# aviadlevis/bhnerf

Hardware: AMD Instinct MI355X
Metric: train ray-samples/sec, 128x128x64-sample image-plane recovery (higher is better)
Workload: dtype bf16

## Files before the change

bhnerf_amd/csrc/fused_bwd.hip:

```cpp
#include <climits>
#include <utility>
#include <type_traits>
#include "fused_common.h"
#include "bwd_common.h"

static constexpr int JOB1_W = 13;
static constexpr int JOBL_W = 7;
static constexpr int GA0C_DIST = 4;
static constexpr int TAPED_DIST = 7;
static constexpr int T8_NBUF = 4;

template <int W, class Pol>
struct BwdGeom {
    static constexpr int MT = W / 32;
    static constexpr int TILE_BYTES = 2 * Pol::FRAG_BYTES;
    static constexpr int TAPE_TILE = Pol::TAPE8 ? 1024 : TILE_BYTES;
    static constexpr int NTMAX = MT + 2;
    static constexpr int SLAB_FLOATS = (MT + 1) * NTMAX * 1024;
    static constexpr int WR = (MT >= 4) ? 4 : MT;
    static constexpr int WC = Pol::NWAVES / WR >= 1 ? Pol::NWAVES / WR : 1;
    static constexpr int WRR = (Pol::NWAVES < WR) ? Pol::NWAVES : WR;
    static constexpr int WCC = Pol::NWAVES / WRR;
    static constexpr int MPW = (MT + WRR - 1) / WRR;
    static constexpr int NPW_ALL = (NTMAX + WCC - 1) / WCC;
    static constexpr int SWEEP = (Pol::NWAVES <= 4) ? NTMAX : 5;
    static constexpr int NPASS = (NPW_ALL + SWEEP - 1) / SWEEP;
    static constexpr int NPW = (NPW_ALL + NPASS - 1) / NPASS;
    static constexpr int GROUP_BYTES = Pol::TAPE8 ? MT * TAPE_TILE + (MT + 1) * TILE_BYTES : (2 * MT + 1) * TILE_BYTES;
    static constexpr int GROUP_BYTES_LAST2 = GROUP_BYTES + 1024;
    static constexpr int RING_DIST_TAPED = (Pol::ELEM_BYTES == 2) ? TAPED_DIST : 3;
    static constexpr int NBUF = (Pol::ELEM_BYTES == 2) ? ((160 * 1024) / GROUP_BYTES >= 4 ? 4 : 3) : 2;
    static constexpr int NPIECE = GROUP_BYTES / 1024;
    static constexpr int PPW = (NPIECE + Pol::NWAVES - 1) / Pol::NWAVES;
};

enum { EMIT_NO_STORE = 1,
       EMIT_OFF = 2 };
template <class Pol>
struct TapeEmit {
    static constexpr int LDS_BYTES = 2 * Pol::FRAG_BYTES;
    const char *table;
    DEVI void init(char *lds) {
        table = lds;
        if (Pol::ELEM_BYTES != 2 && threadIdx.x < 64) {
            const int lane = threadIdx.x, n = lane & 31, h = lane >> 5;
            typename Pol::frag id[2];
#pragma unroll
            for (int s = 0; s < 2; ++s) {
#pragma unroll
                for (int j = 0; j < 8; ++j) Pol::set(id[s], j, phi16(h, j) + 16 * s == n ? 1.f : 0.f);
                if constexpr (Pol::ELEM_BYTES == 2) {
                    *reinterpret_cast<typename Pol::frag *>(lds + s * Pol::FRAG_BYTES + lane * 16) = id[s];
                } else {
#pragma unroll
                    for (int hf = 0; hf < 2; ++hf) {
                        f32x4 v;
#pragma unroll
                        for (int e = 0; e < 4; ++e) v[e] = Pol::get(id[s], 4 * hf + e);
                        *reinterpret_cast<f32x4 *>(lds + s * Pol::FRAG_BYTES + hf * 1024 + lane * 16) = v;
                    }
                }
            }
        }
    }
    DEVI void load_id(typename Pol::frag (&id)[2]) const {
        const int lane = threadIdx.x & 63;
        id[0] = Pol::lds_frag(table, 0, lane);
        id[1] = Pol::lds_frag(table, 1, lane);
    }
    static DEVI f32x16 transpose(const typename Pol::frag &f0, const typename Pol::frag &f1, const typename Pol::frag (&id)[2]) {
        f32x16 t = {};
        t = Pol::mma(f0, id[0], t);
        t = Pol::mma(f1, id[1], t);
        return t;
    }
    static DEVI void store(char *dst, const f32x16 &t) {
        const int lane = threadIdx.x & 63;
        typename Pol::frag o[2];
#pragma unroll
        for (int s = 0; s < 2; ++s)
#pragma unroll
            for (int j = 0; j < 8; ++j) Pol::set(o[s], j, t[8 * s + j]);
        if constexpr (Pol::ELEM_BYTES == 2) {
#pragma unroll
            for (int s = 0; s < 2; ++s) __builtin_nontemporal_store(o[s], reinterpret_cast<typename Pol::frag *>(dst + s * 1024 + lane * 16));
        } else {
#pragma unroll
            for (int s = 0; s < 2; ++s)
#pragma unroll
                for (int hf = 0; hf < 2; ++hf) {
                    f32x4 v;
#pragma unroll
                    for (int e = 0; e < 4; ++e) v[e] = Pol::get(o[s], 4 * hf + e);
                    __builtin_nontemporal_store(v, reinterpret_cast<f32x4 *>(dst + s * 2048 + hf * 1024 + lane * 16));
                }
        }
    }
    static DEVI int native_off(int s) {
        const int lane = threadIdx.x & 63, pt = lane & 31, h = lane >> 5;
        return 16 * (pt & 3) + 128 * s + 64 * h + 256 * (pt >> 2);
    }
    static DEVI void store_native(char *dst, const typename Pol::frag &f0, const typename Pol::frag &f1, int flags = 0) {
        if (!(flags & EMIT_NO_STORE)) {
            __builtin_nontemporal_store(f0, reinterpret_cast<typename Pol::frag *>(dst + native_off(0)));
            __builtin_nontemporal_store(f1, reinterpret_cast<typename Pol::frag *>(dst + native_off(1)));
        } else asm volatile("" ::"v"(f0), "v"(f1));
    }
    DEVI void emit(char *dst, const typename Pol::frag &f0, const typename Pol::frag &f1) const {
        if constexpr (Pol::ELEM_BYTES == 2) {
            store_native(dst, f0, f1);
        } else {
            typename Pol::frag id[2];
            load_id(id);
            store(dst, transpose(f0, f1, id));
        }
    }
};

DEVI long long uniform64(long long v) {
    const unsigned lo = __builtin_amdgcn_readfirstlane((unsigned)v), hi = __builtin_amdgcn_readfirstlane((unsigned)((unsigned long long)v >> 32));
    return (long long)(((unsigned long long)hi << 32) | lo);
}

DEVI int tr_lane_off() {
    const int lane = threadIdx.x & 63, g = lane >> 4, li = lane & 15, q = li >> 2, pp = li & 3;
    return 256 * (g >> 1) + 16 * q + 128 * (g & 1) + 64 * (pp & 1) + 8 * (pp >> 1);
}
DEVI bf16x8 tr_frag(const char *tile, int s, int trl) {
    typedef s16x4 __attribute__((address_space(3))) * lds_v4;
    typedef short s16x8 __attribute__((ext_vector_type(8)));
    const char *a = tile + 1024 * s + trl;
    const s16x4 lo = __builtin_amdgcn_ds_read_tr16_b64_v4i16((lds_v4)(a));
    const s16x4 hi = __builtin_amdgcn_ds_read_tr16_b64_v4i16((lds_v4)(a + 512));
    const s16x8 v = __builtin_shufflevector(lo, hi, 0, 1, 2, 3, 4, 5, 6, 7);
    return __builtin_bit_cast(bf16x8, v);
}

struct Raw8 { u32x2 lo, hi; };
DEVI int tr8_lane_off() {
    const int lane = threadIdx.x & 63, g = lane >> 4, li = lane & 15, tsel = g & 1, kh = g >> 1;
    return 1024 * tsel + 128 * (kh ^ tsel) + 32 * (li >> 2) + 8 * (li & 3);
}
DEVI Raw8 tr8_read(const char *pair, int s2, int tr8) {
    typedef s16x4 __attribute__((address_space(3))) * lds_v4;
    Raw8 r;
    r.lo = __builtin_bit_cast(u32x2, __builtin_amdgcn_ds_read_tr16_b64_v4i16((lds_v4)(pair + 512 * s2 + tr8)));
    r.hi = __builtin_bit_cast(u32x2, __builtin_amdgcn_ds_read_tr16_b64_v4i16((lds_v4)(pair + 512 * s2 + 256 + tr8)));
    return r;
}
struct Pair8 { u32x2 a, b; };
DEVI Pair8 tr8_sort(const Raw8 &r) {
    Pair8 p;
    p.a = (u32x2){__builtin_amdgcn_perm(r.lo[1], r.lo[0], 0x06040200u), __builtin_amdgcn_perm(r.hi[1], r.hi[0], 0x06040200u)};
    p.b = (u32x2){__builtin_amdgcn_perm(r.lo[1], r.lo[0], 0x07050301u), __builtin_amdgcn_perm(r.hi[1], r.hi[0], 0x07050301u)};
    return p;
}
DEVI bf16x8 widen8(const u32x2 &f, float scale) {
    typedef __bf16 b2 __attribute__((ext_vector_type(2)));
    const b2 a0 = __builtin_amdgcn_cvt_scalef32_pk_bf16_fp8(f[0], scale, false), a1 = __builtin_amdgcn_cvt_scalef32_pk_bf16_fp8(f[0], scale, true);
    const b2 a2 = __builtin_amdgcn_cvt_scalef32_pk_bf16_fp8(f[1], scale, false), a3 = __builtin_amdgcn_cvt_scalef32_pk_bf16_fp8(f[1], scale, true);
    return (bf16x8){a0[0], a0[1], a1[0], a1[1], a2[0], a2[1], a3[0], a3[1]};
}
DEVI void tr8_widen(const Raw8 &r, float scale, bf16x8 &fa, bf16x8 &fb) {
    const Pair8 p = tr8_sort(r);
    fa = widen8(p.a, scale);
    fb = widen8(p.b, scale);
}
DEVI f32x16 mma8(const u32x2 &a, const u32x2 &b, f32x16 c) {
    return __builtin_amdgcn_mfma_f32_32x32x16_fp8_fp8(__builtin_bit_cast(long, a), __builtin_bit_cast(long, b), c, 0, 0, 0);
}
__host__ __device__ static inline int t8_feature(int t, int n) {
    const int i = n & 15, hh = i >> 3, s = (i >> 2) & 1, j = 2 * (i & 3) + (t & 1);
    return 32 * ((t & ~1) + (n >> 4)) + 16 * s + 8 * (j >> 2) + 4 * hh + (j & 3);
}

// ... 669 lines not shown
    const int wr = wv % WRR, wc = wv / WRR;
    const bool wave_works = wr * MPW < mtA;
    float *slab = A.f.slabs + (long long)blockIdx.x * BG::SLAB_FLOATS;
    constexpr int PA = out_job ? TB / 1024 : MT * TB / 1024, PH = has_h ? MT * TB / 1024 : 0, PE = has_enc ? TB / 1024 : 0;
    using Stream = TapeStream<Pol::NWAVES, PA, PH, PE, 0, OFF_H, OFF_E, 0>;
    constexpr int PPW = Stream::PPW;
    const Stream stream(srcA, strideA, srcH, (long long)MT * TB, srcE, TB, nullptr, 0, wv);

    for (int pass = 0; pass < NPASS; ++pass) {
        const int nbase = wc * NPWJ + pass * NPW;
        int boff[NPW];
#pragma unroll
        for (int ni = 0; ni < NPW; ++ni) {
            const int n = nbase + ni;
            boff[ni] = (n < nH) ? OFF_H + n * TB : (has_enc ? OFF_E : OFF_H);
        }
        const bool has_tiles = nbase < nB;
        const bool bias_rows = wc == 0 && pass == 0;
        float bsum[MPW];
#pragma unroll
        for (int mi = 0; mi < MPW; ++mi) bsum[mi] = 0.f;
        f32x16 acc[MPW][NPW];
#pragma unroll
        for (int mi = 0; mi < MPW; ++mi)
#pragma unroll
            for (int ni = 0; ni < NPW; ++ni) {
                if constexpr (AGPR) {
                    const f32x16 z = {};
                    acc[mi][ni] = __builtin_amdgcn_mfma_f32_32x32x2f32(0.f, 0.f, z, 0, 0, 0);
                } else {
#pragma unroll
                    for (int r = 0; r < 16; ++r) acc[mi][ni][r] = 0.f;
                }
            }
        __syncthreads();
        auto load_b = [&](const char *gp, int t) -> frag {
            if constexpr (TR) return tr_frag(gp + boff[t % NPW], t / NPW, trl);
            else return Pol::lds_frag(gp + boff[t % NPW], t / NPW, lane);
        };
        auto load_a = [&](const char *tile, int s2) -> frag {
            if constexpr (TR) return tr_frag(tile, s2, trl);
            else return Pol::lds_frag(tile, s2, lane);
        };
        auto compute_group = [&](const char *gp) {
            constexpr int NTOT = 2 * NPW, AHEAD = (Pol::ELEM_BYTES == 2) ? 2 : 1;
            if constexpr (AGPR) {
#pragma unroll
                for (int mi = 0; mi < MPW; ++mi)
#pragma unroll
                    for (int ni = 0; ni < NPW && ni < NPIN; ++ni) asm volatile("" : "+a"(acc[mi][ni]));
            }
            frag af[2][MPW];
#pragma unroll
            for (int s = 0; s < 2; ++s)
#pragma unroll
                for (int mi = 0; mi < MPW; ++mi) {
                    af[s][mi] = load_a(gp + (wr * MPW + mi) * TB, s);
                    if (bias_rows) bsum[mi] = Pol::sum8(af[s][mi], bsum[mi]);
                }
            frag bq[AHEAD + 1];
#pragma unroll
            for (int t = 0; t < AHEAD && t < NTOT; ++t) bq[t] = load_b(gp, t);
#pragma unroll
            for (int t = 0; t < NTOT; ++t) {
                if (t + AHEAD < NTOT) bq[(t + AHEAD) % (AHEAD + 1)] = load_b(gp, t + AHEAD);
                __builtin_amdgcn_sched_barrier(0);
                const int s = t / NPW, ni = t % NPW;
                const frag bnow = bq[t % (AHEAD + 1)];
#pragma unroll
                for (int mi = 0; mi < MPW; ++mi) acc[mi][ni] = Pol::mma(af[s][mi], bnow, acc[mi][ni]);
                __builtin_amdgcn_sched_barrier(0);
            }
        };
        {
            constexpr int NBUF = BG::NBUF;
            auto issue = [&](long long q, char *buf) { stream.issue(q < q1 ? q : q1 - 1, buf); };
            constexpr int INFLIGHT = NBUF - 2;
            if (q0 < q1) {
#pragma unroll
                for (int j = 0; j < NBUF - 1; ++j) issue(q0 + j, smem + j * GB);
                int it = 0;
                for (long long q = q0; q < q1; ++q) {
                    asm volatile("s_waitcnt vmcnt(%0)" ::"n"(INFLIGHT * PPW) : "memory");
                    __builtin_amdgcn_s_barrier();
                    asm volatile("" ::: "memory");
                    const int nx = (it == 0) ? NBUF - 1 : it - 1;
                    issue(q + NBUF - 1, smem + nx * GB);
                    if (wave_works && has_tiles) compute_group(smem + it * GB);
                    it = (it == NBUF - 1) ? 0 : it + 1;
                }
                asm volatile("s_waitcnt vmcnt(0)" ::: "memory");
            }
        }
#pragma unroll
        for (int mi = 0; mi < MPW; ++mi)
#pragma unroll
            for (int ni = 0; ni < NPW; ++ni) {
                const int m = wr * MPW + mi, n = nbase + ni;
                if (m >= mtA || n >= nB || n >= (wc + 1) * NPWJ) continue;
                if constexpr (AGPR) { if (ni < NPIN) asm volatile("" : "+a"(acc[mi][ni])); }
                float *tp = slab + (long long)(m * BG::NTMAX + n) * 1024;
#pragma unroll
                for (int g4 = 0; g4 < 4; ++g4) {
                    f32x4 v;
#pragma unroll
                    for (int e = 0; e < 4; ++e) v[e] = acc[mi][ni][4 * g4 + e];
                    f32x4 *dst = reinterpret_cast<f32x4 *>(tp + g4 * 256 + lane * 4);
                    if (A.accumulate) {
                        const f32x4 old = *dst;
#pragma unroll
                        for (int e = 0; e < 4; ++e) v[e] += old[e];
                    }
                    *dst = v;
                }
                __builtin_amdgcn_sched_barrier(0);
            }
        if (bias_rows) {
#pragma unroll
            for (int mi = 0; mi < MPW; ++mi) {
                const int m = wr * MPW + mi;
                float v = bsum[mi] + __shfl_xor(bsum[mi], 32, 64);
                if (m < mtA && lane < 32) {
                    const int hh = (lane >> 2) & 1, r = (lane & 3) + 4 * (lane >> 3);
                    float *dst = slab + (long long)(m * BG::NTMAX + nB) * 1024 + (r >> 2) * 256 + (32 * hh) * 4 + (r & 3);
                    if (A.accumulate) v += *dst;
                    *dst = v;
                }
            }
        }
    }
}


template <int W, class Pol, int JT, bool LAST = false, bool OUTENC = false>
DEVI void dw_body2(const BwdArgs &A, int job, char *smem) {
    using BG = BwdGeom<W, Pol>;
    using frag = typename Pol::frag;
    static_assert(Pol::ELEM_BYTES == 2 && JT != JT_OUT && JT != JT_OUTSKIP, "bf16 jobs of layers 0 .. depth-1");
    static_assert(!LAST || JT == JT_HIDDEN || JT == JT_SKIP, "LAST: hidden / skip job");
    static_assert(!OUTENC || LAST, "OUTENC: a LAST job");
    static_assert(BG::NBUF == 4, "ring of four group buffers");
    constexpr int MT = BG::MT, TB = BG::TILE_BYTES, TT = BG::TAPE_TILE;
    constexpr bool T8 = Pol::TAPE8;
    constexpr bool has_h = JT != JT_FIRST, make_h = JT == JT_HIDDEN1, enc_extra = JT == JT_SKIP;
    static_assert(!T8 || !OUTENC, "8-bit tape: even depths / no skip into the output layer");
    constexpr int OFF_H = MT * TT, OFF_E = T8 ? OFF_H + (make_h ? MT * TB : MT * TT) : 2 * MT * TB, OFF_D32 = OFF_E + TB;
    constexpr int GB = OFF_D32 + (LAST ? 1024 : 0);
    static_assert(T8 || (OFF_D32 == BG::GROUP_BYTES && GB == (LAST ? BG::GROUP_BYTES_LAST2 : BG::GROUP_BYTES)), "group image");
    static_assert(GB <= BG::GROUP_BYTES + 1024, "group image larger than the host's LDS budget");
    constexpr int NB = (T8 && !make_h) ? T8_NBUF : 4;
    static_assert((NB & (NB - 1)) == 0 && NB >= 4 && NB * GB <= 160 * 1024, "ring size");
    constexpr int nH = has_h ? MT : 0, nB = nH + ((JT == JT_FIRST || JT == JT_SKIP) ? 1 : 0);
    constexpr int nBr = has_h ? MT : 1;
    constexpr int WRR = BG::WRR, WCC = BG::WCC;
    constexpr int MPW = (MT + WRR - 1) / WRR, NPW = (nBr + WCC - 1) / WCC;
    static_assert(NPW <= 5, "one sweep");
    constexpr bool F8 = T8 && has_h && !make_h;
    static_assert(!T8 || MPW == 2, "8-bit tape: the A tiles come in pairs (width 256)");
    static_assert(!F8 || NPW % 2 == 0, "8-bit tape: the B tiles come in pairs (width 256)");
    constexpr int ME = (MPW + WCC - 1) / WCC;
    constexpr int NTOT = 2 * NPW;
    const int tid = threadIdx.x, lane = tid & 63, wv = __builtin_amdgcn_readfirstlane(tid >> 6);
    const int trl = tr_lane_off();
    const int tr8 = tr8_lane_off();
    float scaleA = 1.f;
    if constexpr (T8 && !LAST) scaleA = __builtin_bit_cast(float, __builtin_amdgcn_readfirstlane(__builtin_bit_cast(int, A.t8[job])));
    if constexpr (F8 && LAST) {
        const float v = A.t8[job];
        scaleA = __builtin_bit_cast(float, __builtin_amdgcn_readfirstlane(__builtin_bit_cast(int, (v > 0.f && v < __builtin_inff()) ? v : 1.f)));
    }
    const int nwg = A.wg_begin[job + 1] - A.wg_begin[job];
    const int kb = blockIdx.x - A.wg_begin[job];
    const long long q0 = uniform64(A.t.NQ * kb / nwg), q1 = uniform64(A.t.NQ * (kb + 1) / nwg);
    const char *srcA = LAST ? A.tape + A.t.h_off[job + 1] : A.tape + A.t.ga_off[job];
    const char *srcD = A.tape + A.t.dout_off;
    const char *srcH = has_h ? A.tape + A.t.h_off[job] : nullptr;
    const char *srcE = A.tape + (make_h ? A.t.encp_off : A.t.enc_off);
    const int wr = wv % WRR, wc = wv / WRR;
    const int nbase = wc * NPW;
    const bool works = wr * MPW < MT && nbase < nBr;
    char *w0_lds = smem + NB * GB;
    float *b0_lds = reinterpret_cast<float *>(w0_lds + 2 * MT * Pol::FRAG_BYTES);
    if constexpr (make_h) {
        const char *w0 = A.f.packed + A.f.fwd_off;
        for (int i = tid; i < 2 * MT * Pol::FRAG_BYTES / 16; i += Pol::NTHREADS)
            reinterpret_cast<u32x4 *>(w0_lds)[i] = reinterpret_cast<const u32x4 *>(w0)[i];
        for (int i = tid; i < W; i += Pol::NTHREADS) b0_lds[i] = reinterpret_cast<const float *>(A.f.packed + A.f.bias_off)[i];
    }
    struct HIn { frag e0, e1, w0, w1; float b; };
    auto make_h_read = [&](const char *gp) {
        HIn in;
        in.e0 = Pol::lds_frag(gp + OFF_E, 0, lane); in.e1 = Pol::lds_frag(gp + OFF_E, 1, lane);
        const int t = wv < MT ? wv : 0;
        in.w0 = Pol::lds_frag(w0_lds, 2 * t, lane); in.w1 = Pol::lds_frag(w0_lds, 2 * t + 1, lane);
        in.b = b0_lds[32 * t + (lane & 31)];
        return in;
    };
    auto make_h_mma = [&](const HIn &in) {
        f32x16 acc;
#pragma unroll
        for (int r = 0; r < 16; ++r) acc[r] = in.b;
        acc = Pol::mma(in.e0, in.w0, acc);
        acc = Pol::mma(in.e1, in.w1, acc);
        return acc;
    };
    auto make_h_write = [&](char *gp, const f32x16 &acc) {
        if (wv < MT) {
            frag o[2];
            unsigned unused = 0;
#pragma unroll
            for (int r = 0; r < 16; r += 2) Pol::relu_pair(o[r >> 3], (r & 7) >> 1, r >> 1, acc[r], acc[r + 1], unused);
#pragma unroll
            for (int s2 = 0; s2 < 2; ++s2) *reinterpret_cast<frag *>(gp + OFF_H + wv * TB + s2 * Pol::FRAG_BYTES + lane * 16) = o[s2];
        }
    };
    float wout_r[MPW];
    if constexpr (LAST) {
#pragma unroll
        for (int mi = 0; mi < MPW; ++mi) {
            const int f = T8 ? t8_feature(wr * MPW + mi, lane & 31) : 32 * (wr * MPW + mi) + (lane & 31);
            wout_r[mi] = f < W ? reinterpret_cast<const float *>(A.f.packed + A.f.wout_off)[f] : 0.f;
        }
    }
    float *slab = A.f.slabs + (long long)blockIdx.x * BG::SLAB_FLOATS;

    int boff[NPW];
#pragma unroll
    for (int ni = 0; ni < NPW; ++ni) {
        const int n = nbase + ni;
        boff[ni] = has_h ? OFF_H + (n < nH ? n : 0) * (F8 ? TT : TB) : OFF_E;
    }
    const bool bias_rows = wc == 0;
    const bool out_bias_wave = LAST && wr == 0 && wc == 0;
    f32x16 acc[MPW][NPW], acc_e[ME];
    float bsum[MPW], orow[ME], bout = 0.f, oenc = 0.f;
#pragma unroll
    for (int mi = 0; mi < MPW; ++mi) {
        bsum[mi] = 0.f;
#pragma unroll
        for (int ni = 0; ni < NPW; ++ni)
#pragma unroll
            for (int r = 0; r < 16; ++r) acc[mi][ni][r] = 0.f;
    }
#pragma unroll
    for (int e = 0; e < ME; ++e) {
        orow[e] = 0.f;
#pragma unroll
        for (int r = 0; r < 16; ++r) acc_e[e][r] = 0.f;
    }

    struct AState { frag af[2][MPW]; f32x4 da[2], db[2]; frag ef[2]; u32x2 a8[2][MPW]; };
    auto load_b = [&](const char *gp, int t) -> frag {
        if constexpr (make_h) return Pol::lds_frag(gp + boff[t % NPW], t / NPW, lane);
        else return tr_frag(gp + boff[t % NPW], t / NPW, trl);
    };
    constexpr int NPH = NPW / 2 > 0 ? NPW / 2 : 1;
    auto load_braw = [&](const char *gp, int u) -> Raw8 { return tr8_read(gp + boff[2 * (u % NPH)], u / NPH, tr8); };
    auto a_load = [&](const char *gp, AState &st) {
#pragma unroll
        for (int s2 = 0; s2 < 2; ++s2) {
#pragma unroll
            for (int mi = 0; mi < MPW; ++mi) {
                if constexpr (T8) {
                    if (mi == 0) {
                        const Raw8 raw = tr8_read(gp + (wr * MPW) * TT, s2, tr8);
                        st.af[s2][0] = __builtin_bit_cast(frag, (u32x4){raw.lo[0], raw.lo[1], raw.hi[0], raw.hi[1]});
                    }
                } else st.af[s2][mi] = tr_frag(gp + (wr * MPW + mi) * TB, s2, trl);
            }
            if constexpr (LAST) {
                const float *d32 = reinterpret_cast<const float *>(gp + OFF_D32) + 16 * s2 + 4 * (lane >> 5);
                st.da[s2] = *reinterpret_cast<const f32x4 *>(d32);
                st.db[s2] = *reinterpret_cast<const f32x4 *>(d32 + 8);
                if constexpr (OUTENC) st.ef[s2] = tr_frag(gp + OFF_E, s2, trl);
            }
        }
    };
    auto a_prep = [&](AState &st, int k, bool live) {
        const int s2 = k / MPW, mi = k % MPW;
        if constexpr (F8) {
            if (mi == 0) {
                const u32x4 rw = __builtin_bit_cast(u32x4, st.af[s2][0]);
                Raw8 raw;
                raw.lo = (u32x2){rw[0], rw[1]}; raw.hi = (u32x2){rw[2], rw[3]};
                const Pair8 pr = tr8_sort(raw);
                st.a8[s2][0] = pr.a; st.a8[s2][1] = pr.b;
            }
            if constexpr (!LAST) {
                if (bias_rows || (enc_extra && (mi % WCC) == wc)) st.af[s2][mi] = widen8(st.a8[s2][mi], scaleA);
            } else {
                typedef float f32x2 __attribute__((ext_vector_type(2)));
                typedef short s16x2 __attribute__((ext_vector_type(2)));
                const f32x4 da = st.da[s2], db = st.db[s2];
                const u32x2 h8 = st.a8[s2][mi];
                const bool my_row = (mi % WCC) == wc;
                u32x2 d8;
#pragma unroll
                for (int i = 0; i < 2; ++i) {
                    const f32x4 d4 = i == 0 ? da : db;
                    s16x2 r = {0, 0};
                    r = __builtin_amdgcn_cvt_scalef32_pk_fp8_f32(r, d4[0], d4[1], scaleA, false);
                    r = __builtin_amdgcn_cvt_scalef32_pk_fp8_f32(r, d4[2], d4[3], scaleA, true);
                    d8[i] = __builtin_bit_cast(unsigned, r);
                }
                if (my_row) {
                    const frag hb = widen8(h8, 1.f);
                    float o = 0.f;
#pragma unroll
                    for (int i = 0; i < 4; ++i) {
                        const f32x2 dd = {i < 2 ? da[2 * i] : db[2 * i - 4], i < 2 ? da[2 * i + 1] : db[2 * i - 3]};
                        const typename Pol::bf16x2 dpk = {(__bf16)dd[0], (__bf16)dd[1]};
                        const typename Pol::bf16x2 hp = {hb[2 * i], hb[2 * i + 1]};
                        o = __builtin_amdgcn_fdot2_f32_bf16(hp, dpk, o, false);
                    }
                    if (live) orow[mi / WCC] += o;
                }
                u32x2 g8;
#pragma unroll
                for (int i = 0; i < 2; ++i) {
                    const unsigned t = (h8[i] + 0x7f7f7f7fu) & 0x80808080u;
                    g8[i] = d8[i] & (t | (t - (t >> 7)));
                }
                st.a8[s2][mi] = g8;
                if (bias_rows || (enc_extra && (mi % WCC) == wc)) st.af[s2][mi] = widen8(g8, scaleA);
                if (live && out_bias_wave && mi == 0) bout += (da[0] + da[1]) + (da[2] + da[3]) + (db[0] + db[1]) + (db[2] + db[3]);
            }
            if (live && bias_rows) bsum[mi] = Pol::sum8(st.af[s2][mi], bsum[mi]);
            return;
        } else if constexpr (T8) {
            if (mi == 0) {
                const u32x4 rw = __builtin_bit_cast(u32x4, st.af[s2][0]);
                Raw8 raw;
                raw.lo = (u32x2){rw[0], rw[1]}; raw.hi = (u32x2){rw[2], rw[3]};
                tr8_widen(raw, scaleA, st.af[s2][0], st.af[s2][1]);
            }
        }
        if constexpr (LAST) {
            typedef float f32x2 __attribute__((ext_vector_type(2)));
            typedef short i16x2 __attribute__((ext_vector_type(2)));
            const f32x4 da = st.da[s2], db = st.db[s2];
            const frag rawf = st.af[s2][mi];
            const u32x4 raw = __builtin_bit_cast(u32x4, rawf);
            u32x4 ga;
            float o = 0.f;
            const bool my_row = (mi % WCC) == wc;
#pragma unroll
            for (int i = 0; i < 4; ++i) {
                const f32x2 dd = {i < 2 ? da[2 * i] : db[2 * i - 4], i < 2 ? da[2 * i + 1] : db[2 * i - 3]};
                const typename Pol::bf16x2 dpk = {(__bf16)dd[0], (__bf16)dd[1]};
                const typename Pol::bf16x2 hp = {rawf[2 * i], rawf[2 * i + 1]};
                if (my_row) o = __builtin_amdgcn_fdot2_f32_bf16(hp, dpk, o, false);
                if constexpr (OUTENC) {
                    if (live && out_bias_wave && mi == 0) {
                        const typename Pol::bf16x2 ep = {st.ef[s2][2 * i], st.ef[s2][2 * i + 1]};
                        oenc = __builtin_amdgcn_fdot2_f32_bf16(ep, dpk, oenc, false);
                    }
                }
                const unsigned sgn = raw[i] + 0x7fff7fffu;
                const i16x2 on = __builtin_bit_cast(i16x2, sgn) >> (i16x2){15, 15};
                ga[i] = __builtin_bit_cast(unsigned, dpk) & __builtin_bit_cast(unsigned, on);
            }
            st.af[s2][mi] = __builtin_bit_cast(frag, ga);
            if (live && my_row) orow[mi / WCC] += o;
            if (live && out_bias_wave && mi == 0) bout += (da[0] + da[1]) + (da[2] + da[3]) + (db[0] + db[1]) + (db[2] + db[3]);
        }
        if (live && bias_rows) bsum[mi] = Pol::sum8(st.af[s2][mi], bsum[mi]);
    };
    constexpr int NPREP = 2 * MPW;
    constexpr int T_PREP = NTOT > 3 ? 3 : NTOT - 1;
    auto mma_phase = [&](const char *gp, const AState &cur, const frag (&bc)[2], const char *gnext, AState &nx, frag (&bn)[2],
                         bool live_next) {
        frag bq[3], benc;
        if constexpr (F8) {
            constexpr int NPAIR = NTOT / 2;
            u32x4 bcur = __builtin_bit_cast(u32x4, bc[0]), bnx = bcur;
            Raw8 rnext, rawn;
            if (NPAIR > 1) rnext = load_braw(gp, 1);
#pragma unroll
            for (int t = 0; t < NTOT; ++t) {
                const int u = t >> 1, e = t & 1;
                if (e == 0 && u + 1 < NPAIR) {
                    const Pair8 pr = tr8_sort(rnext);
                    bnx = (u32x4){pr.a[0], pr.a[1], pr.b[0], pr.b[1]};
                    if (u + 2 < NPAIR) rnext = load_braw(gp, u + 2);
                }
                if (enc_extra && (t % NPW) == (NPW >= 2 ? NPW - 2 : 0)) benc = tr_frag(gp + OFF_E, t / NPW, trl);
                if (t == 0) a_load(gnext, nx);
                __builtin_amdgcn_sched_barrier(0);
                const int s2 = t / NPW, ni = t % NPW;
                const u32x2 bnow = e == 0 ? (u32x2){bcur[0], bcur[1]} : (u32x2){bcur[2], bcur[3]};
#pragma unroll
                for (int mi = 0; mi < MPW; ++mi) acc[mi][ni] = mma8(cur.a8[s2][mi], bnow, acc[mi][ni]);
                if constexpr (enc_extra) {
                    if (ni == NPW - 1) {
#pragma unroll
                        for (int mi = 0; mi < MPW; ++mi)
                            if ((mi % WCC) == wc) acc_e[mi / WCC] = Pol::mma(cur.af[s2][mi], benc, acc_e[mi / WCC]);
                    }
                }
#pragma unroll
                for (int k = 0; k < NPREP; ++k)
                    if (t == (T_PREP + k < NTOT ? T_PREP + k : NTOT - 1)) a_prep(nx, k, live_next);
                if (t == (NTOT >= 2 ? NTOT - 2 : 0)) rawn = load_braw(gnext, 0);
                if (t == NTOT - 1) {
                    const Pair8 pr = tr8_sort(rawn);
                    bn[0] = __builtin_bit_cast(frag, (u32x4){pr.a[0], pr.a[1], pr.b[0], pr.b[1]});
                }
                __builtin_amdgcn_sched_barrier(0);
                if (e == 1) bcur = bnx;
            }
            return;
        }
        if constexpr (make_h) {
            bq[0] = load_b(gp, 0);
            if (NTOT > 1) bq[1] = load_b(gp, 1);
        } else {
            bq[0] = bc[0]; bq[1] = bc[1];
        }
#pragma unroll
        for (int t = 0; t < NTOT; ++t) {
            if (t + 2 < NTOT) bq[(t + 2) % 3] = load_b(gp, t + 2);
            if (enc_extra && (t % NPW) == (NPW >= 2 ? NPW - 2 : 0)) benc = tr_frag(gp + OFF_E, t / NPW, trl);
            if (t == 0) a_load(gnext, nx);
            __builtin_amdgcn_sched_barrier(0);
            const int s2 = t / NPW, ni = t % NPW;
#pragma unroll
            for (int mi = 0; mi < MPW; ++mi) acc[mi][ni] = Pol::mma(cur.af[s2][mi], bq[t % 3], acc[mi][ni]);
            if constexpr (enc_extra) {
                if (ni == NPW - 1) {
#pragma unroll
                    for (int mi = 0; mi < MPW; ++mi)
                        if ((mi % WCC) == wc) acc_e[mi / WCC] = Pol::mma(cur.af[s2][mi], benc, acc_e[mi / WCC]);
                }
            }
#pragma unroll
            for (int k = 0; k < NPREP; ++k)
                if (t == (T_PREP + k < NTOT ? T_PREP + k : NTOT - 1)) a_prep(nx, k, live_next);
            if constexpr (!make_h) {
                if (t == (NTOT >= 2 ? NTOT - 2 : 0)) bn[0] = load_b(gnext, 0);
                if (t == NTOT - 1) bn[1] = load_b(gnext, NTOT > 1 ? 1 : 0);
            }
            __builtin_amdgcn_sched_barrier(0);
        }
    };

    constexpr int PA = MT * TT / 1024, PH = (has_h && !make_h) ? MT * TT / 1024 : 0,
                  PE = (JT == JT_FIRST || JT == JT_SKIP || make_h || OUTENC) ? TB / 1024 : 0, PD = LAST ? 1 : 0;
    using Stream = TapeStream<Pol::NWAVES, PA, PH, PE, PD, OFF_H, OFF_E, OFF_D32>;
    constexpr int PPW = Stream::PPW;
    const Stream stream(srcA, (long long)MT * TT, srcH, (long long)MT * TT, srcE, TB, srcD, A.t.dout_stride, wv);
    auto issue = [&](long long q, char *buf) { stream.issue(q < q1 ? q : q1 - 1, buf); };
    __syncthreads();
    if (q0 < q1) {
        AState sa, sb;
        frag ba[2], bb[2];
#pragma unroll
        for (int j = 0; j < NB - 1; ++j) issue(q0 + j, smem + j * GB);
        asm volatile("s_waitcnt vmcnt(%0)" ::"n"((NB - 2) * PPW) : "memory");
        __builtin_amdgcn_s_barrier();
        asm volatile("" ::: "memory");
        if constexpr (make_h) make_h_write(smem, make_h_mma(make_h_read(smem)));
        if (works) {
            a_load(smem, sa);
#pragma unroll
            for (int k = 0; k < NPREP; ++k) a_prep(sa, k, true);
            if constexpr (F8) {
                const Pair8 pr = tr8_sort(load_braw(smem, 0));
                ba[0] = __builtin_bit_cast(frag, (u32x4){pr.a[0], pr.a[1], pr.b[0], pr.b[1]});
            } else if constexpr (!make_h) { ba[0] = load_b(smem, 0); ba[1] = load_b(smem, NTOT > 1 ? 1 : 0); }
        }
        auto body = [&](AState &cur, AState &nx, frag (&bc)[2], frag (&bn)[2], long long q, int it) {
            asm volatile("s_waitcnt vmcnt(%0)" ::"n"((NB - 3) * PPW) : "memory");
            if constexpr (make_h) asm volatile("s_waitcnt lgkmcnt(0)" ::: "memory");
            __builtin_amdgcn_s_barrier();
            asm volatile("" ::: "memory");
            issue(q + NB - 1, smem + ((it + NB - 1) & (NB - 1)) * GB);
            const char *gp = smem + it * GB;
            char *gnext = smem + ((it + 1) & (NB - 1)) * GB;
            const bool live_next = q + 1 < q1;
            f32x16 hacc = {};
            if constexpr (make_h) hacc = make_h_mma(make_h_read(gnext));
            if (works) mma_phase(gp, cur, bc, gnext, nx, bn, live_next);
            if constexpr (make_h) {
                if (live_next) make_h_write(gnext, hacc);
            }
        };
        int it = 0;
        for (long long q = q0; q < q1;) {
            body(sa, sb, ba, bb, q, it);
            ++q; it = (it + 1) & (NB - 1);
            if (q >= q1) break;
            body(sb, sa, bb, ba, q, it);
            ++q; it = (it + 1) & (NB - 1);
        }
        asm volatile("s_waitcnt vmcnt(0)" ::: "memory");
    }
    const float *wout_g = reinterpret_cast<const float *>(A.f.packed + A.f.wout_off);
    auto flush_tile = [&](int m, int n, const f32x16 &t, bool enc_tile = false) {
        float *tp = slab + (long long)(m * BG::NTMAX + n) * 1024;
#pragma unroll
        for (int g4 = 0; g4 < 4; ++g4) {
            f32x4 v;
#pragma unroll
            for (int e = 0; e < 4; ++e) v[e] = t[4 * g4 + e];
            if constexpr (LAST && T8) {
#pragma unroll
                for (int e = 0; e < 4; ++e) v[e] *= (F8 && n < nBr && !enc_tile ? scaleA : 1.f) * wout_g[t8_feature(m, 8 * g4 + 4 * (lane >> 5) + e)];
            } else if constexpr (F8) {
                if (!enc_tile) {
#pragma unroll
                    for (int e = 0; e < 4; ++e) v[e] *= scaleA;
                }
            } else if constexpr (LAST) {
                const f32x4 w4 = *reinterpret_cast<const f32x4 *>(wout_g + 32 * m + 8 * g4 + 4 * (lane >> 5));
#pragma unroll
                for (int e = 0; e < 4; ++e) v[e] *= w4[e];
            }
            f32x4 *dst = reinterpret_cast<f32x4 *>(tp + g4 * 256 + lane * 4);
            if (A.accumulate) {
                const f32x4 old = *dst;
#pragma unroll
                for (int e = 0; e < 4; ++e) v[e] += old[e];
            }
            *dst = v;
        }
    };
    auto flush_column0 = [&](int m, int n, float v, bool on) {
        v += __shfl_xor(v, 32, 64);
        if (on && lane < 32) {
            const int hh = (lane >> 2) & 1, r = (lane & 3) + 4 * (lane >> 3);
            float *dst = slab + (long long)(m * BG::NTMAX + n) * 1024 + (r >> 2) * 256 + (32 * hh) * 4 + (r & 3);
            if (A.accumulate) v += *dst;
            *dst = v;
        }
    };
#pragma unroll
    for (int mi = 0; mi < MPW; ++mi) {
        const int m = wr * MPW + mi;
#pragma unroll
        for (int ni = 0; ni < NPW; ++ni) {
            const int n = nbase + ni;
            if (m < MT && n < nBr) flush_tile(m, n, acc[mi][ni]);
        }
        if (enc_extra && (mi % WCC) == wc && m < MT) flush_tile(m, nH, acc_e[mi / WCC], true);
        flush_column0(m, nB, LAST ? bsum[mi] * wout_r[mi] : bsum[mi], bias_rows && m < MT);
        if constexpr (LAST) {
            float v = orow[mi / WCC] + __shfl_xor(orow[mi / WCC], 32, 64);
            if ((mi % WCC) == wc && m < MT && lane < 32) {
                float *dst = slab + (long long)(MT * BG::NTMAX + m) * 1024 + lane * 4;
                if (A.accumulate) v += *dst;
                *dst = v;
            }
        }
    }
    if constexpr (LAST) {
        float v = bout + __shfl_xor(bout, 32, 64);
        if (out_bias_wave && lane == 0) {
            float *dst = slab + (long long)(MT * BG::NTMAX + MT + (OUTENC ? 1 : 0)) * 1024;
            if (A.accumulate) v += *dst;
            *dst = v;
        }
        if constexpr (OUTENC) {
            float ve = oenc + __shfl_xor(oenc, 32, 64);
            if (out_bias_wave && lane < 32) {
                float *dst = slab + (long long)(MT * BG::NTMAX + MT) * 1024 + lane * 4;
                if (A.accumulate) ve += *dst;
                *dst = ve;
            }
        }
    }
}

template <int W, class Pol>
__global__ __launch_bounds__(Pol::NTHREADS) __attribute__((amdgpu_waves_per_eu(Pol::NWAVES == 4 ? 1 : (W <= 128 ? 4 : 2)))) void dw_kernel(BwdArgs A) {
    extern __shared__ __attribute__((aligned(16))) char smem[];
    const int depth = A.f.depth;
    clock_stamp(A.f.clk, BHN_CLK_DW, 0);
    int job = 0;
    while (job < depth && (int)blockIdx.x >= A.wg_begin[job + 1]) ++job;
    if constexpr (Pol::ELEM_BYTES == 2) {
        const bool out_skip = (A.f.skip_mask >> depth) & 1;
        if (job == depth) {
            if (out_skip) dw_body<W, Pol, JT_OUTSKIP>(A, job, smem);
            else dw_body<W, Pol, JT_OUT>(A, job, smem);
        } else if (job == depth - 1 && A.t.drop_ga) {
            if constexpr (Pol::TAPE8) {
                if ((A.f.skip_mask >> job) & 1) dw_body2<W, Pol, JT_SKIP, true>(A, job, smem);
                else dw_body2<W, Pol, JT_HIDDEN, true>(A, job, smem);
            } else if ((A.f.skip_mask >> job) & 1) {
                if (out_skip) dw_body2<W, Pol, JT_SKIP, true, true>(A, job, smem);
                else dw_body2<W, Pol, JT_SKIP, true>(A, job, smem);
            } else {
                if (out_skip) dw_body2<W, Pol, JT_HIDDEN, true, true>(A, job, smem);
                else dw_body2<W, Pol, JT_HIDDEN, true>(A, job, smem);
            }
        } else if (job == 0) dw_body2<W, Pol, JT_FIRST>(A, job, smem);
        else if ((A.f.skip_mask >> job) & 1) dw_body2<W, Pol, JT_SKIP>(A, job, smem);
        else if (job == 1 && A.t.drop_h1) dw_body2<W, Pol, JT_HIDDEN1>(A, job, smem);
        else dw_body2<W, Pol, JT_HIDDEN>(A, job, smem);
    } else {
        if (job == depth) {
            if ((A.f.skip_mask >> depth) & 1) dw_body<W, Pol, JT_OUTSKIP>(A, job, smem);
            else dw_body<W, Pol, JT_OUT>(A, job, smem);
        } else if (job == 0) dw_body<W, Pol, JT_FIRST>(A, job, smem);
        else if ((A.f.skip_mask >> job) & 1) dw_body<W, Pol, JT_SKIP>(A, job, smem);
        else dw_body<W, Pol, JT_HIDDEN>(A, job, smem);
    }
    clock_stamp(A.f.clk, BHN_CLK_DW, 1);
}

template <int W, class Pol>
struct ReduceGeom {
    using BG = BwdGeom<W, Pol>;
    static __host__ __device__ int n_b(int l, unsigned skip_mask) { return (l >= 1 ? BG::MT : 0) + ((l == 0 || ((skip_mask >> l) & 1)) ? 1 : 0); }
    static __host__ __device__ int rows(int l, int depth) { return l == depth ? 1 : BG::MT; }
    static __host__ __device__ int blocks(int depth, unsigned skip_mask) {
        int n = 0;
        for (int l = 0; l <= depth; ++l) n += rows(l, depth) * (n_b(l, skip_mask) + 1);
        return n;
    }
};

__global__ __launch_bounds__(256) void chain_slab_stage1(BwdArgs A, int mt, int per) {
    const int tile = blockIdx.x, s0 = blockIdx.y * per, s1 = (s0 + per < A.n_chain_wg) ? s0 + per : A.n_chain_wg;
// ... 72 lines not shown
__global__ __launch_bounds__(1024) void t8_dmax_kernel(float *st, const float *dimages, long long n) {
    __shared__ float red[16];
    float m = 0.f;
    for (long long i = blockIdx.x * 1024ll + threadIdx.x; i < n; i += (long long)gridDim.x * 1024) m = __builtin_fmaxf(m, __builtin_fabsf(dimages[i]));
#pragma unroll
    for (int o = 32; o >= 1; o >>= 1) m = __builtin_fmaxf(m, __shfl_xor(m, o, 64));
    if ((threadIdx.x & 63) == 0) red[threadIdx.x >> 6] = m;
    __syncthreads();
    if (threadIdx.x == 0) {
        float d = 0.f;
        for (int i = 0; i < 16; ++i) d = __builtin_fmaxf(d, red[i]);
        if (!(d < __builtin_inff())) d = __builtin_inff();
        atomicMax(reinterpret_cast<unsigned *>(st) + 25, __float_as_uint(d));
    }
}
__global__ void t8_prepare_kernel(float *st, int nl, int fresh) {
    if (threadIdx.x != 0) return;
    float d = st[24];
    if (fresh) {
        d = st[25];
        st[25] = 0.f;
        if (!(d < __builtin_inff())) d = 0.f;
        st[24] = d;
    }
    for (int l = 0; l < nl; ++l) {
        const float a = st[16 + l] * d;
        if (a > 0.f && a < __builtin_inff()) {
            int e;
            const float mant = frexpf(a * (16.f / 448.f), &e);
            if (mant == 0.5f) --e;
            e = e < -100 ? -100 : e > 100 ? 100 : e;
            st[l] = ldexpf(1.f, e);
        } else if (!(st[l] > 0.f && st[l] < __builtin_inff())) st[l] = 1.f;
    }
}
__global__ void t8_update_kernel(float *st, int nl) {
    const int l = threadIdx.x;
    if (l >= nl) return;
    unsigned *bits = reinterpret_cast<unsigned *>(st);
    const float a = __uint_as_float(bits[8 + l]), d = st[24];
    if (a > 0.f && a < __builtin_inff() && d > 0.f) st[16 + l] = a / d;
    bits[8 + l] = 0u;
}
__global__ void t8_open_kernel(float *st) {
    if (threadIdx.x < 8) { st[threadIdx.x] = 0x1p60f; reinterpret_cast<unsigned *>(st)[8 + threadIdx.x] = 0u; }
}

int fused_fill_args(const bhn_model *m, int32_t mode, const void *packed, const bhn_geom *geom,
                    const bhn_frames *fr, bool need_w, FusedArgs *a, MlpShape *s, int nwaves);

static size_t align_up(size_t v, size_t a) { return (v + a - 1) / a * a; }

template <int W, class Pol>
static constexpr bool ga0_chain_ok(int depth) {
    return Pol::ELEM_BYTES == 2 && !Pol::TAPE8 && W / 32 == Pol::NWAVES && depth >= 3;
}

template <int W, class Pol>
static void tape_layout(int depth, bool layer1_takes_enc, bool last_takes_enc, long long NQ, TapeLayout *t) {
    using BG = BwdGeom<W, Pol>;
    memset(t, 0, sizeof(*t));
    t->NQ = NQ;
    t->drop_h1 = Pol::ELEM_BYTES == 2 && depth >= 2 && !layer1_takes_enc;
    long long off = 0;
    const long long per_tensor = NQ * BG::MT * (long long)BG::TAPE_TILE;
    for (int l = 1; l <= depth; ++l) {
        if (l == 1 && t->drop_h1) { t->h_off[l] = -1; continue; }
        t->h_off[l] = off; off += per_tensor;
    }
    if (t->drop_h1) { t->encp_off = off; off += NQ * (long long)BG::TILE_BYTES; }
    t->drop_ga = bhn_folds_wout(Pol::MODE, depth);
    t->ga0_chain = ga0_chain_ok<W, Pol>(depth) && t->drop_ga;
    for (int l = 0; l < depth; ++l) {
        if ((l == depth - 1 && t->drop_ga) || (l == 0 && t->ga0_chain)) { t->ga_off[l] = -1; continue; }
        t->ga_off[l] = off; off += per_tensor;
    }
    t->lin_stride = per_tensor;
    {
        const int lmin = t->drop_h1 ? 2 : 1;
        t->h_lin = (lmin <= depth ? t->h_off[lmin] : 0) - lmin * per_tensor;
        t->ga_lin = t->ga0_chain ? t->ga_off[1] - per_tensor : t->ga_off[0];
    }
    t->enc_off = off; off += NQ * (long long)BG::TILE_BYTES;
    t->dout_stride = t->drop_ga ? 128 : BG::TILE_BYTES;
    t->dout_off = off; off += NQ * t->dout_stride;
    t->mask_off = off; off += NQ * (long long)depth * ((BG::MT + 1) / 2) * 256;
    t->e_off = off; off += NQ * 128;
    off = (long long)align_up((size_t)off + 1024, 256);
    t->total = off;
}

template <int W, class Pol>
static void tape_traffic(const MlpShape &s, const TapeLayout &t, int64_t *o) {
    using BG = BwdGeom<W, Pol>;
    const long long TT = BG::TAPE_TILE, TB = BG::TILE_BYTES, MT = BG::MT, MW = (MT + 1) / 2, depth = s.depth;
    long long fw = 0, cw = 0, cr = 0, dr = 0;
    if (t.fused128) {
        fw = (depth - 2) * MT * TB + MW * 256 + TB + 128;
        dr = fw + 128;
        cw = 128; cr = 128;
    } else {
        fw = TB + (t.drop_h1 ? TB : 0) + depth * MW * 256 + 128;
        for (int l = 1; l <= depth; ++l) if (t.h_off[l] >= 0) fw += MT * TT;
        for (int l = 0; l < depth; ++l) if (t.ga_off[l] >= 0) cw += MT * TT;
        cw += t.dout_stride;
        cr = depth * MW * 256 + 128 + (t.ga0_chain ? TB : 0);
        const int last_job = t.drop_ga ? (int)depth - 1 : (int)depth;
        for (int l = 0; l <= last_job; ++l) {
            if (l == 0) { if (!t.ga0_chain) dr += MT * TT + TB; continue; }
            if (l == depth) { dr += t.dout_stride + MT * TT + (s.skip_in[l] ? TB : 0); continue; }
            const bool last = l == depth - 1 && t.drop_ga;
            dr += last ? MT * TT + 1024 : MT * TT;
            dr += (l == 1 && t.drop_h1) ? TB : MT * TT;
            if (s.skip_in[l] || (last && s.skip_in[depth])) dr += TB;
        }
    }
    o[0] = fw; o[1] = cw; o[2] = cr; o[3] = dr;
    o[4] = (t.drop_h1 ? 1 : 0) | (t.drop_ga ? 2 : 0) | (t.ga0_chain ? 4 : 0) | (t.fused128 ? 8 : 0) | (t.drop_hd ? 16 : 0);
}

static constexpr size_t T8_STATE_BYTES = 256;

template <int W, class Pol>
struct BwdPlan {
    using Kernel = void (*)(BwdArgs);
    int depth;
    bool skip1, skip_last;
    bool f128;
    bool ga0c;
    int nwf;
    bool x12;
    size_t slab_dw_bytes, slab_bytes, tape_off;
    int wg_begin[BHN_MAX_LAYERS + 2];
    size_t lds_fixed, lds_taped, lds_fwd, lds_chn, lds_dw, res_fwd;
    bool rf, rch;
    Kernel k_fwd, k_chn, kdw;
    void layout(long long NQ, TapeLayout *t) const {
        if (f128) bwd128_tape_layout(depth, NQ, t);
        else tape_layout<W, Pol>(depth, skip1, skip_last, NQ, t);
    }
};

template <int W, class Pol>
static void dw_job_split(const MlpShape &s, const TapeLayout &t, int grid_dw, int *wg_begin) {
    using BG = BwdGeom<W, Pol>;
    const int depth = s.depth;
    double work[BHN_MAX_LAYERS + 1], tot = 0;
    const int last_job = t.drop_ga ? depth - 1 : depth;
    for (int l = 0; l <= depth; ++l) {
        const int mtA = (l == depth) ? 0 : BG::MT;
        int nB = (l >= 1 ? BG::MT : 0) + ((l == 0 || s.skip_in[l]) ? 1 : 0);
        if (l == 1 && t.drop_h1) nB = JOB1_W * BG::MT / 8;
        work[l] = (double)(mtA + nB) + 0.5;
        if (l == depth - 1 && t.drop_ga) work[l] += (Pol::TAPE8 ? 12 : JOBL_W) * BG::MT / 8.0;
        if constexpr (Pol::ELEM_BYTES == 4) {
            const int a_tiles = (l == depth) ? 1 : BG::MT;
            const int wrr = (l == depth) ? 1 : BG::WRR, wcc = Pol::NWAVES / wrr;
            const double tp = (double)((a_tiles + wrr - 1) / wrr) * ((nB + wcc - 1) / wcc);
            const double kib = (double)(a_tiles + nB) * BG::TILE_BYTES / 1024.0;
            work[l] = (tp > 0.075 * kib ? tp : 0.075 * kib) + 0.1;
        }
        if (l > last_job) work[l] = 0;
        if (t.ga0_chain && l == 0) work[l] = 0;
        tot += work[l];
    }
    int used = 0;
    wg_begin[0] = 0;
    for (int l = 0; l <= depth; ++l) {
        int n = (int)(grid_dw * work[l] / tot);
        if (n < 1) n = 1;
        if (l == last_job) n = grid_dw - used;
        if (n < 1) n = 1;
        if (l > last_job || (t.ga0_chain && l == 0)) n = 0;
        used += n;
        wg_begin[l + 1] = used;
    }
}

template <int W, class Pol>
static void bwd_plan(const MlpShape &s, long long groups_per_frame, int ncu, int Sx, BwdPlan<W, Pol> *p) {
    using BG = BwdGeom<W, Pol>;
    using PK = Pack<W, Pol>;
    constexpr bool CAN_RES = W <= 128;
    constexpr bool CAN_X = W == 128 && Pol::ELEM_BYTES == 2 && !Pol::TAPE8;
    using FPol = std::conditional_t<CAN_X, PolBF16X, Pol>;
    constexpr bool CAN_GA0C = ga0_chain_ok<W, Pol>(3);
    const int depth = s.depth;
    p->depth = depth;
    p->skip1 = depth >= 2 && s.skip_in[1];
    p->skip_last = depth >= 2 && s.skip_in[depth - 1];
    p->f128 = bwd128_supported(Pol::MODE, W, depth);
    p->ga0c = !p->f128 && ga0_chain_ok<W, Pol>(depth) && bhn_folds_wout(Pol::MODE, depth);
    p->nwf = bhn_fwd_tile_groups(Pol::MODE, W, depth, groups_per_frame);
    p->x12 = CAN_X && p->nwf == FPol::NWAVES;
    p->slab_dw_bytes = align_up(p->f128 ? bwd128_slab_bytes(ncu) : (size_t)ncu * BG::SLAB_FLOATS * 4, 256);
    p->slab_bytes = p->slab_dw_bytes + (p->ga0c ? align_up((size_t)ncu * BG::MT * 4096, 256) : 0);
    p->tape_off = p->slab_bytes + (Pol::TAPE8 ? T8_STATE_BYTES : 0);
    TapeLayout t;
    p->layout(1, &t);
    dw_job_split<W, Pol>(s, t, ncu, p->wg_begin);
    p->lds_fixed = ((size_t)depth * W + 32) * 4 + 128 + W * 4 + (Pol::ELEM_BYTES == 2 ? 0 : 2 * Pol::FRAG_BYTES) + RaySum<Pol::NWAVES>::bytes(Sx);
    p->lds_taped = (size_t)(BG::RING_DIST_TAPED + 1) * PK::CHUNK_BYTES + p->lds_fixed;
    const size_t lds_fwd_encr = (size_t)(BG::RING_DIST_TAPED + 1) * PK::KS * Pol::FRAG_BYTES + p->lds_fixed + EncBlock<W, Pol>::BYTES;
    p->lds_dw = (size_t)BG::NBUF * BG::GROUP_BYTES + (t.drop_h1 ? (size_t)2 * BG::MT * Pol::FRAG_BYTES + W * 4 : 0);
    if (t.drop_ga && (size_t)BG::NBUF * BG::GROUP_BYTES_LAST2 > p->lds_dw) p->lds_dw = (size_t)BG::NBUF * BG::GROUP_BYTES_LAST2;
    if constexpr (Pol::TAPE8) {
        const size_t deep = (size_t)T8_NBUF * (2 * BG::MT * BG::TAPE_TILE + BG::TILE_BYTES + 1024);
        if (deep > p->lds_dw) p->lds_dw = deep;
    }
    p->res_fwd = (size_t)PK::fwd_chunks(depth) * PK::CHUNK_BYTES + p->lds_fixed;
    const size_t res_chn = (size_t)PK::bwd_chunks(depth) * PK::CHUNK_BYTES + p->lds_fixed;
    p->rf = CAN_RES && p->res_fwd <= 160 * 1024;
    p->rch = CAN_RES && res_chn <= 160 * 1024;
    const size_t res_fwd_x = p->res_fwd - RaySum<Pol::NWAVES>::bytes(Sx) + RaySum<FPol::NWAVES>::bytes(Sx);
    const size_t chain_rows_bytes = 128 + (size_t)W * 4;
    p->lds_fwd = (p->x12 ? res_fwd_x : p->rf ? p->res_fwd : (EncBlock<W, Pol>::ON ? lds_fwd_encr : p->lds_taped)) - chain_rows_bytes;
    const size_t lds_ga0c = (size_t)(GA0C_DIST + 1) * PK::KS * Pol::FRAG_BYTES + p->lds_fixed + (size_t)4 * Pol::NWAVES * BG::TILE_BYTES;
    p->lds_chn = p->ga0c ? lds_ga0c : p->rch ? res_chn : p->lds_taped;
    p->k_fwd = p->x12 ? chain_kernel<W, FPol, 3, MODE_FWD_TRAIN, CAN_RES>
             : p->rf  ? chain_kernel<W, Pol, 3, MODE_FWD_TRAIN, CAN_RES> : chain_kernel<W, Pol, 3, MODE_FWD_TRAIN, false>;
    p->k_chn = p->ga0c ? chain_kernel<W, Pol, 3, MODE_CHAIN, false, CAN_GA0C>
             : p->rch  ? chain_kernel<W, Pol, 3, MODE_CHAIN, CAN_RES> : chain_kernel<W, Pol, 3, MODE_CHAIN, false>;
    p->kdw = dw_kernel<W, Pol>;
}

enum BwdPath { BWD_GENERAL, BWD_F32, BWD_BF16, BWD_BF16_T8 };

static int bwd_path(int32_t mode, const MlpShape &s, BwdPath *path) {
    const bool t8 = (mode & 0xff) == BHN_BF16_T8 && bhn_norm_mode(mode) == BHN_BF16;
    BHN_CHECK_ARG(mode == BHN_F32 || mode == BHN_BF16 || t8, "bad mode %d", mode);
    if (t8 && (s.general || s.width_true != 256 || s.depth < 3 || s.skip_in[s.depth])) {
        bhn_set_error("BHN_BF16_T8 (8-bit tape) is built for net_width 256, net_depth >= 3, posenc_deg <= 4 and no skip-concat "
                      "into the output layer (got %d x %d, posenc_deg %d); use BHN_BF16", s.depth, s.width_true, s.deg);
        return BHN_EUNSUPPORTED;
    }
    *path = s.general ? BWD_GENERAL : t8 ? BWD_BF16_T8 : mode == BHN_BF16 ? BWD_BF16 : BWD_F32;
    return BHN_OK;
}

template <class F>
static int with_bwd_kernels(BwdPath path, int width, F &&f) {
    if (path == BWD_BF16_T8) return f(std::integral_constant<int, 256>(), PolBF16T8());
    return path == BWD_BF16 ? bhn_with_width<PolBF16>(width, f) : bhn_with_width<PolF32>(width, f);
}

template <class Pol>
static int t8_scales(const BwdArgs &A, bool calibrate, const float *dimages, int depth, hipStream_t st) {
    if constexpr (Pol::TAPE8) {
        const long long npx = (long long)A.f.B * A.f.Sx * A.f.R;
        if (calibrate) BHN_HIP(hipMemsetAsync(A.t8, 0, T8_STATE_BYTES, st));
        hipLaunchKernelGGL(t8_dmax_kernel, dim3((unsigned)(npx >= 65536 ? 64 : (npx + 1023) / 1024)), dim3(1024), 0, st, A.t8, dimages, npx);
        hipLaunchKernelGGL(t8_prepare_kernel, dim3(1), dim3(64), 0, st, A.t8, depth, 1);
        BHN_HIP(hipGetLastError());
    }
    return BHN_OK;
}
template <class Pol>
static int t8_calibrate(const BwdArgs &A, void (*k_chn)(BwdArgs), long long grid, size_t lds_chn, int depth, hipStream_t st) {
    if constexpr (Pol::TAPE8) {
        hipLaunchKernelGGL(t8_open_kernel, dim3(1), dim3(64), 0, st, A.t8);
        hipLaunchKernelGGL(k_chn, dim3((unsigned)grid), dim3(Pol::NTHREADS), lds_chn, st, A);
        hipLaunchKernelGGL(t8_update_kernel, dim3(1), dim3(64), 0, st, A.t8, depth);
        hipLaunchKernelGGL(t8_prepare_kernel, dim3(1), dim3(64), 0, st, A.t8, depth, 0);
        BHN_HIP(hipGetLastError());
    }
    return BHN_OK;
}
template <class Pol>
static void t8_update(const BwdArgs &A, int depth, hipStream_t st) {
    if constexpr (Pol::TAPE8) hipLaunchKernelGGL(t8_update_kernel, dim3(1), dim3(64), 0, st, A.t8, depth);
}

enum { RUN_RECOMPUTE, RUN_FWD_TRAIN, RUN_BWD_TAPE };

template <int W, class Pol>
static int frames_per_pass(int what, const BwdPlan<W, Pol> &p, long long groups_per_frame, int B, size_t workspace_bytes, long long *fpp) {
    TapeLayout t;
    p.layout(groups_per_frame, &t);
    if (workspace_bytes < p.tape_off + (size_t)t.total) {
        bhn_set_error("render_bwd workspace too small: %zu bytes, need >= %zu (slabs %zu + one frame of tape %lld)",
                      workspace_bytes, p.tape_off + (size_t)t.total, p.slab_bytes, t.total);
        return BHN_EWORKSPACE;
    }
    *fpp = 1;
    while (*fpp < B) {
        p.layout(groups_per_frame * (*fpp + 1), &t);
        if (p.tape_off + (size_t)t.total > workspace_bytes) break;
        ++*fpp;
    }
    if (what != RUN_RECOMPUTE && *fpp < B) {
        bhn_set_error("the recorded-tape path needs a workspace for all %d frames at once (%zu bytes given); "
                      "use bhn_render_fwd + bhn_render_bwd, which iterate over frame groups", B, workspace_bytes);
        return BHN_EWORKSPACE;
    }
    return BHN_OK;
}

template <int W, class Pol>
static int bwd_pass(int what, const BwdPlan<W, Pol> &p, const BwdArgs &A, int pass, long long grid, int ncu, bool t8_cal,
                    int *nslabs128, hipStream_t st, void *const *events, int n_events) {
    auto mark = [&](int i) -> hipError_t {
        return (events && i < n_events && events[i] && pass == 0) ? hipEventRecord((hipEvent_t)events[i], st) : hipSuccess;
    };
    if (what != RUN_FWD_TRAIN) BHN_HIP(mark(0));
    if (what != RUN_BWD_TAPE) {
        hipLaunchKernelGGL(p.k_fwd, dim3((unsigned)grid), dim3((unsigned)p.nwf * 64u), p.lds_fwd, st, A);
        BHN_HIP(hipGetLastError());
// ... 242 lines not shown
```

Baseline: 706.8 million.

## Give each wave a full A-row strip in the LAST bf16 weight-gradient job

For the last bf16 (non-8-bit-tape) weight-gradient job with as many row tiles as waves, every wave now owns one A row tile and sweeps all B column tiles (WRR = NWAVES, WCC = 1). The B-fragment prefetch ring deepens from 3 to 4 slots, and the next group's first three B fragments are preloaded. The host's per-job workgroup split uses a smaller weight for this job because its per-wave work changes. The aim is to reuse A fragments across more MMAs and hide more LDS latency, at the cost of more accumulator tiles and registers per wave, which the new 10-tile assert bounds.

Result: faster. 716.7 million (median of 6 runs) (+1.4%).

```diff
diff --git a/bhnerf_amd/csrc/fused_bwd.hip b/bhnerf_amd/csrc/fused_bwd.hip
--- a/bhnerf_amd/csrc/fused_bwd.hip
+++ b/bhnerf_amd/csrc/fused_bwd.hip
@@ -6,6 +6,7 @@
 
 static constexpr int JOB1_W = 13;
 static constexpr int JOBL_W = 7;
+static constexpr int JOBL_ROWS_W = 3;
 static constexpr int GA0C_DIST = 4;
 static constexpr int TAPED_DIST = 7;
 static constexpr int T8_NBUF = 4;
@@ -21,6 +22,7 @@
     static constexpr int WC = Pol::NWAVES / WR >= 1 ? Pol::NWAVES / WR : 1;
     static constexpr int WRR = (Pol::NWAVES < WR) ? Pol::NWAVES : WR;
     static constexpr int WCC = Pol::NWAVES / WRR;
+    static constexpr bool LAST_ROWS = Pol::ELEM_BYTES == 2 && !Pol::TAPE8 && MT == Pol::NWAVES;
     static constexpr int MPW = (MT + WRR - 1) / WRR;
     static constexpr int NPW_ALL = (NTMAX + WCC - 1) / WCC;
     static constexpr int SWEEP = (Pol::NWAVES <= 4) ? NTMAX : 5;
@@ -996,13 +998,15 @@
     static_assert((NB & (NB - 1)) == 0 && NB >= 4 && NB * GB <= 160 * 1024, "ring size");
     constexpr int nH = has_h ? MT : 0, nB = nH + ((JT == JT_FIRST || JT == JT_SKIP) ? 1 : 0);
     constexpr int nBr = has_h ? MT : 1;
-    constexpr int WRR = BG::WRR, WCC = BG::WCC;
+    constexpr bool ROWS8 = LAST && BG::LAST_ROWS;
+    constexpr int WRR = ROWS8 ? Pol::NWAVES : BG::WRR, WCC = Pol::NWAVES / WRR;
     constexpr int MPW = (MT + WRR - 1) / WRR, NPW = (nBr + WCC - 1) / WCC;
-    static_assert(NPW <= 5, "one sweep");
     constexpr bool F8 = T8 && has_h && !make_h;
     static_assert(!T8 || MPW == 2, "8-bit tape: the A tiles come in pairs (width 256)");
     static_assert(!F8 || NPW % 2 == 0, "8-bit tape: the B tiles come in pairs (width 256)");
     constexpr int ME = (MPW + WCC - 1) / WCC;
+    static_assert(MPW * NPW + ME <= 10, "one sweep: at most 10 accumulator tiles per wave (two waves per SIMD)");
+    constexpr int BQD = ROWS8 ? 4 : 3, NBC = BQD - 1;
     constexpr int NTOT = 2 * NPW;
     const int tid = threadIdx.x, lane = tid & 63, wv = __builtin_amdgcn_readfirstlane(tid >> 6);
     const int trl = tr_lane_off();
@@ -1020,7 +1024,7 @@
     const char *srcD = A.tape + A.t.dout_off;
     const char *srcH = has_h ? A.tape + A.t.h_off[job] : nullptr;
     const char *srcE = A.tape + (make_h ? A.t.encp_off : A.t.enc_off);
-    const int wr = wv % WRR, wc = wv / WRR;
+    const int wr = WCC == 1 ? wv : wv % WRR, wc = WCC == 1 ? 0 : wv / WRR;
     const int nbase = wc * NPW;
     const bool works = wr * MPW < MT && nbase < nBr;
     char *w0_lds = smem + NB * GB;
@@ -1212,9 +1216,9 @@
     };
     constexpr int NPREP = 2 * MPW;
     constexpr int T_PREP = NTOT > 3 ? 3 : NTOT - 1;
-    auto mma_phase = [&](const char *gp, const AState &cur, const frag (&bc)[2], const char *gnext, AState &nx, frag (&bn)[2],
+    auto mma_phase = [&](const char *gp, const AState &cur, const frag (&bc)[NBC], const char *gnext, AState &nx, frag (&bn)[NBC],
                          bool live_next) {
-        frag bq[3], benc;
+        frag bq[BQD], benc;
         if constexpr (F8) {
             constexpr int NPAIR = NTOT / 2;
             u32x4 bcur = __builtin_bit_cast(u32x4, bc[0]), bnx = bcur;
@@ -1258,18 +1262,21 @@
         if constexpr (make_h) {
             bq[0] = load_b(gp, 0);
             if (NTOT > 1) bq[1] = load_b(gp, 1);
+        } else if constexpr (NBC == 2) {
+            bq[0] = bc[0]; bq[1] = bc[1];
         } else {
-            bq[0] = bc[0]; bq[1] = bc[1];
+#pragma unroll
+            for (int j = 0; j < NBC; ++j) bq[j] = bc[j];
         }
 #pragma unroll
         for (int t = 0; t < NTOT; ++t) {
-            if (t + 2 < NTOT) bq[(t + 2) % 3] = load_b(gp, t + 2);
+            if (t + BQD - 1 < NTOT) bq[(t + BQD - 1) % BQD] = load_b(gp, t + BQD - 1);
             if (enc_extra && (t % NPW) == (NPW >= 2 ? NPW - 2 : 0)) benc = tr_frag(gp + OFF_E, t / NPW, trl);
             if (t == 0) a_load(gnext, nx);
             __builtin_amdgcn_sched_barrier(0);
             const int s2 = t / NPW, ni = t % NPW;
 #pragma unroll
-            for (int mi = 0; mi < MPW; ++mi) acc[mi][ni] = Pol::mma(cur.af[s2][mi], bq[t % 3], acc[mi][ni]);
+            for (int mi = 0; mi < MPW; ++mi) acc[mi][ni] = Pol::mma(cur.af[s2][mi], bq[t % BQD], acc[mi][ni]);
             if constexpr (enc_extra) {
                 if (ni == NPW - 1) {
 #pragma unroll
@@ -1281,8 +1288,14 @@
             for (int k = 0; k < NPREP; ++k)
                 if (t == (T_PREP + k < NTOT ? T_PREP + k : NTOT - 1)) a_prep(nx, k, live_next);
             if constexpr (!make_h) {
-                if (t == (NTOT >= 2 ? NTOT - 2 : 0)) bn[0] = load_b(gnext, 0);
-                if (t == NTOT - 1) bn[1] = load_b(gnext, NTOT > 1 ? 1 : 0);
+                if constexpr (NBC == 2) {
+                    if (t == (NTOT >= 2 ? NTOT - 2 : 0)) bn[0] = load_b(gnext, 0);
+                    if (t == NTOT - 1) bn[1] = load_b(gnext, NTOT > 1 ? 1 : 0);
+                } else {
+#pragma unroll
+                    for (int j = 0; j < NBC; ++j)
+                        if (t == NTOT - NBC + j) bn[j] = load_b(gnext, j);
+                }
             }
             __builtin_amdgcn_sched_barrier(0);
         }
@@ -1297,7 +1310,7 @@
     __syncthreads();
     if (q0 < q1) {
         AState sa, sb;
-        frag ba[2], bb[2];
+        frag ba[NBC], bb[NBC];
 #pragma unroll
         for (int j = 0; j < NB - 1; ++j) issue(q0 + j, smem + j * GB);
         asm volatile("s_waitcnt vmcnt(%0)" ::"n"((NB - 2) * PPW) : "memory");
@@ -1311,9 +1324,13 @@
             if constexpr (F8) {
                 const Pair8 pr = tr8_sort(load_braw(smem, 0));
                 ba[0] = __builtin_bit_cast(frag, (u32x4){pr.a[0], pr.a[1], pr.b[0], pr.b[1]});
-            } else if constexpr (!make_h) { ba[0] = load_b(smem, 0); ba[1] = load_b(smem, NTOT > 1 ? 1 : 0); }
-        }
-        auto body = [&](AState &cur, AState &nx, frag (&bc)[2], frag (&bn)[2], long long q, int it) {
+            } else if constexpr (!make_h && NBC == 2) { ba[0] = load_b(smem, 0); ba[1] = load_b(smem, NTOT > 1 ? 1 : 0); }
+            else if constexpr (!make_h) {
+#pragma unroll
+                for (int j = 0; j < NBC; ++j) ba[j] = load_b(smem, j);
+            }
+        }
+        auto body = [&](AState &cur, AState &nx, frag (&bc)[NBC], frag (&bn)[NBC], long long q, int it) {
             asm volatile("s_waitcnt vmcnt(%0)" ::"n"((NB - 3) * PPW) : "memory");
             if constexpr (make_h) asm volatile("s_waitcnt lgkmcnt(0)" ::: "memory");
             __builtin_amdgcn_s_barrier();
@@ -1692,7 +1709,7 @@
         int nB = (l >= 1 ? BG::MT : 0) + ((l == 0 || s.skip_in[l]) ? 1 : 0);
         if (l == 1 && t.drop_h1) nB = JOB1_W * BG::MT / 8;
         work[l] = (double)(mtA + nB) + 0.5;
-        if (l == depth - 1 && t.drop_ga) work[l] += (Pol::TAPE8 ? 12 : JOBL_W) * BG::MT / 8.0;
+        if (l == depth - 1 && t.drop_ga) work[l] += (Pol::TAPE8 ? 12 : BG::LAST_ROWS ? JOBL_ROWS_W : JOBL_W) * BG::MT / 8.0;
         if constexpr (Pol::ELEM_BYTES == 4) {
             const int a_tiles = (l == depth) ? 1 : BG::MT;
             const int wrr = (l == depth) ? 1 : BG::WRR, wcc = Pol::NWAVES / wrr;
```
